# MarcKloter/bulletproofs_gadgets

Measured on AMD Instinct MI355X. Metric: R1CS constraints/sec (prove), 2^20-constraint MiMC-Merkle, 1/2/4/8 GPU, higher is better.
Workload: dtype u32

## Files before the change

### bulletproofs_gadgets_amd/csrc/engine.hip

```cpp
#include <hip/hip_runtime.h>
#include <algorithm>
#include <array>
#include <chrono>
#include <cerrno>
#include <cstdio>
#include <cstdlib>
#include <cstring>
#include <atomic>
#include <condition_variable>
#include <deque>
#include <functional>
#include <map>
#include <memory>
#include <mutex>
#include <thread>
#include <sched.h>
#include <fcntl.h>
#include <sys/stat.h>
#include <unistd.h>
#include "engine.hpp"
#include "hip_handles.hpp"
#include "host/fe51.hpp"
#include "host/chain.hpp"
#include "host/fiat_shamir.hpp"
#include "host/csc_work.hpp"
#include "host/verify_wave_plan.hpp"
#include "host/merkle_plan.hpp"
#include "hip/kernels.cuh"

namespace bpg {

#define BPG_LAUNCH_ID(I, id, kernel, grid, block, ...) do { (I).prof_begin(id); hipLaunchKernelGGL(kernel, grid, block, 0, (I).st, __VA_ARGS__); (I).prof_end(id); } while (0)
#define BPG_LAUNCH(I, kernel, grid, block, ...) BPG_LAUNCH_ID(I, KID_##kernel, kernel, grid, block, __VA_ARGS__)
#define BPG_LAUNCH_LDS(I, id, kernel, grid, block, lds, ...) do { (I).prof_begin(id); hipLaunchKernelGGL(kernel, grid, block, lds, (I).st, __VA_ARGS__); (I).prof_end(id); } while (0)

namespace {

static std::mutex g_table_bytes_mutex;
static std::map<int, uint64_t> g_table_bytes;
static uint64_t table_bytes_held(int device) { std::lock_guard<std::mutex> lk(g_table_bytes_mutex); return g_table_bytes[device]; }
static void table_bytes_add(int device, int64_t delta) { std::lock_guard<std::mutex> lk(g_table_bytes_mutex); g_table_bytes[device] = (uint64_t)((int64_t)g_table_bytes[device] + delta); }
static std::atomic<int> g_proving[64];
struct ProvingGuard {
    std::atomic<int> &c;
    explicit ProvingGuard(int device) : c(g_proving[(unsigned)device & 63u]) { c.fetch_add(1, std::memory_order_relaxed); }
    ~ProvingGuard() { c.fetch_sub(1, std::memory_order_relaxed); }
};
static bool device_shared(int device) { return g_proving[(unsigned)device & 63u].load(std::memory_order_relaxed) > 1; }
struct SharedTables {
    int device = 0; uint64_t cap = 0;
    DevBuf gens;
    std::mutex m;
    std::map<uint32_t, DevBuf> wide;
    std::map<uint32_t, DevBuf> odd;
    std::map<uint64_t, uint64_t> refused;
    ~SharedTables() {
        (void)hipSetDevice(device);
        uint64_t held = 0;
        for (auto &kv : odd) held += kv.second.cap;
        for (auto &kv : wide) held += kv.second.cap;
        table_bytes_add(device, -(int64_t)held);
    }
};
struct MimcConstants {
    int device = 0; DevBuf rc;
    ~MimcConstants() { (void)hipSetDevice(device); }
};
static std::mutex g_mimc_mutex;
void merkle_orphan(DeviceMerkle *t);
static std::map<int, std::weak_ptr<MimcConstants>> g_mimc;
static std::mutex g_tables_mutex;
// ... 127 lines not shown
    void prof_note(int id, double alg_bytes, double act_bytes, double fm) { if (!prof_on(id)) return; prof_alg_bytes[id] += alg_bytes; prof_act_bytes[id] += act_bytes; prof_fm[id] += fm; }
    void prof_collect() {
        if (prof_open.empty()) return;
        HIPCHK(hipStreamSynchronize(st));
        for (ProfRec &r : prof_open) { float ms = 0; HIPCHK(hipEventElapsedTime(&ms, r.a, r.b)); prof_ms[r.id] += ms; prof_count[r.id]++; if ((r.id == KID_k_witness_eval || r.id == KID_k_witness_eval_repeat || r.id == KID_k_witness_eval_join) && prof_wit_ms.size() < 1024) prof_wit_ms.push_back(ms); if ((r.id == KID_k_merkle_level || r.id == KID_k_merkle_top || r.id == KID_k_merkle_level_list || r.id == KID_k_merkle_level_range || r.id == KID_k_merkle_climb) && prof_merkle_ms.size() < 512) prof_merkle_ms.emplace_back(r.id, ms); prof_pool.push_back(std::move(r.a)); prof_pool.push_back(std::move(r.b)); }
        prof_open.clear();
    }
    void prof_reset() { prof_collect(); for (int i = 0; i < KID_COUNT; i++) { prof_ms[i] = 0; prof_count[i] = 0; prof_alg_bytes[i] = prof_act_bytes[i] = prof_fm[i] = 0; } prof_wit_ms.clear(); prof_merkle_ms.clear(); }
    std::shared_ptr<SharedTables> shared;
    const ge_niels *gens = nullptr;
    DevBuf bases, scratch_ext, comp, small_in, small_sc;
    std::shared_ptr<MimcConstants> mimc;
    DevBuf mk_in, mk_out;
    std::vector<DeviceMerkle *> trees;
    DevBuf chk_v, chk_bitmap, chk_report;
    DevBuf ck_first;
    uint32_t check_threshold = CHECK_ROW_THRESHOLD;
    void rowview_build(DeviceCircuit *c);
    void fill_input_slots(DeviceCircuit *c);
    DevBuf arena;
    uint8_t *arena_at(size_t off) const { return arena.as<uint8_t>() + off; }
    bool blocking_waits = false;
    void wait_stream() {
        if (blocking_waits && !shared_now) {
            const double until = now_ms() + 3.0;
            do {
                const hipError_t e = hipStreamQuery(st);
                if (e == hipSuccess) return;
                if (e != hipErrorNotReady) HIPCHK(e);
                for (int k = 0; k < 64; k++) __builtin_ia32_pause();
            } while (now_ms() < until);
        }
        HIPCHK(hipStreamSynchronize(st));
    }
    static size_t al256(size_t x) { return (x + 255) & ~(size_t)255; }
    DevBuf counts, starts, cursor, blocksum, buckets, partial, msm_result, open_keys, medium, wsums, wq_stage, wq_tickets, tile_hist, heavy, plain, starts1;
    uint32_t sweep_blocks_resident = 1024;
    uint32_t msm_cmax = 15;
    uint32_t msm_cmax_shared = 16;
    uint32_t rseg = 8;
    uint32_t lgch = 0;
    bool gens_share = true;
    uint32_t profile = 1;
    bool shared_now = false;
    uint32_t msm_cmin = 2;
    uint32_t wit_waves = 1024;
    uint32_t merge_equal = 1;
    uint32_t merged_last = 0, merged_skipped_last = 0;
    void merge_witness(DeviceCircuit *c, const ge_niels *Gtab, const ge_niels *Htab);
    void merge_build(DeviceCircuit::MergeSet &M, const scm *A, const ge_niels *PA, uint32_t nA, const scm *B, const ge_niels *PB, uint32_t nB);
    double merge_ms_last = 0;
    DevBuf sLR, yinvpow, lv, rv, red_partial, red_out, raw_rng, extras;
    DevBuf stale_flag;
    DevBuf ipa_s, ipa_tabA, ipa_tabB, naf, qsteps, vfy_in, vfy_pts, vfy_ok, vfy_sc, vfy_ch;
    DevBuf vfy_small;
    DevBuf vw_raw, vw_flags, vw_standing, vw_tail1;
    uint32_t cu_count = 256;
    DevBuf tt_bases, tt_table, tt_f, tt_c, tt_partial, grp_c, ped_table, s_parts;
    uint32_t tt_orig_M0 = 0; const void *tt_orig_gens = nullptr;
    ge_pniels *tt_table_p = nullptr;
    void tt_build(const ge_niels *G, const ge_niels *H, const ge_niels *B, uint32_t M0, bool original) {
        const uint32_t npts = 2 * M0 + 1;
        if (original && tt_orig_M0 == M0 && tt_orig_gens == gens) { tt_table_p = tt_table.as<ge_pniels>(); return; }
        const size_t bb = al256((size_t)npts * TT_WINDOWS * sizeof(ge_ext)), tb = (size_t)npts * TT_WINDOWS * TT_MULTS * sizeof(ge_pniels);
        ge_ext *basesp;
        if (original) {
            tt_orig_M0 = 0;
// ... 85 lines not shown
                BPG_LAUNCH((*this), k_normalize_niels, ngrid, dim3(256), base.as<ge_ext>(), tab0, cnt);
                BPG_LAUNCH((*this), k_odd_start_ext, grid, dim3(256), base.as<ge_ext>(), scratch_ext.as<ge_ext>(), dbl.as<ge_ext>(), cnt);
            }
            for (uint32_t m = 1; m < NM; m++) {
                if (m > 1) BPG_LAUNCH((*this), k_odd_step, grid, dim3(256), scratch_ext.as<ge_ext>(), dbl.as<ge_ext>(), cnt);
                BPG_LAUNCH((*this), k_normalize_niels, ngrid, dim3(256), scratch_ext.as<ge_ext>(), tab0 + (size_t)m * cnt, cnt);
            }
        }
        HIPCHK(hipGetLastError());
        HIPCHK(hipStreamSynchronize(st));
        } catch (...) {
            (void)hipStreamSynchronize(st); table_bytes_add(shared->device, -(int64_t)odd.cap);
            throw;
        }
        gens_odd = (shared->odd[key_built] = std::move(odd)).as<ge_niels>();
        return true;
    }
    uint32_t fold_split_max = 65536;
    uint32_t fold_adapt = 1;
    bool shared_variants() const { return fold_adapt == 2 || (fold_adapt == 1 && device_shared(shared->device)); }
    bool fold_quad = true;
    bool fold_quad_w = true;
    bool fold_reg_w = true;
    FoldKnobs fold_knobs() const {
        FoldKnobs k;
        k.fold_wnaf = fold_wnaf; k.fold_split_max = fold_split_max; k.fold_quad = fold_quad; k.fold_quad_w = fold_quad_w; k.fold_reg_w = fold_reg_w; k.shared = shared_now;
        return k;
    }
    bool window_quad = true;
    uint32_t window_quad_blocks = 288;
    uint32_t fold_group = 3;
    uint32_t tt_lg = 12;
    uint32_t tt_orig_lg = 14;
    uint32_t batch_wave_mb = 512;
    DevBuf bt_dev; PinBuf bt_pin;
    uint32_t commit_cpw = 4;
    Event commit_ev;
    PinBuf h_raw, h_small;
    using BlindStream = bpg::BlindStream;
    using ChainWorker = bpg::ChainWorker;
    std::shared_ptr<ChainWorker> chain;
    uint32_t pool_streams = 0;
    uint32_t chain_workers = 1;
    uint32_t chain_lanes = 1;
    std::deque<std::shared_ptr<BlindStream>> blinds;
    std::vector<std::shared_ptr<BlindStream>> slab_owner;
    std::vector<PinBuf> h_blind;
    struct SlabDev { Stream copy_st; DevBuf d; std::vector<Event> ev; };
    static hipEvent_t block_event(const BlindStream &bs, uint64_t k) { return (*static_cast<const std::vector<Event> *>(bs.ev))[k]; }
// ... 14 lines not shown
    }
    void blind_release(const std::shared_ptr<BlindStream> &b) {
        blind_stop(b);
        for (auto it = blinds.begin(); it != blinds.end(); ++it) if (it->get() == b.get()) { blinds.erase(it); break; }
    }
    void blind_cancel() {
        while (!blinds.empty()) { blind_retire(blinds.front()); blinds.pop_front(); }
    }
    void chain_shutdown() {
        blind_cancel();
        if (!chain) return;
        if (!chain->pool) chain->stop();
        chain.reset(); pool_streams = 0;
    }
    uint64_t gens_cap = 0;
    DevBuf gens_load_cached(const std::string &path, uint64_t cap);
    void adopt(const std::shared_ptr<SharedTables> &sp) { shared = sp; gens = sp->gens.as<ge_niels>(); gens_cap = sp->cap; gens_odd = nullptr; }
    void gens_store_cached(const std::string &path, uint64_t cap);

    struct MsmTicket { uint32_t slot, nmsm, W; };
    static constexpr uint32_t WS_SLOTS = 8, WS_SLOT_BYTES = (uint32_t)MSM_WS_SLOT_BYTES;
    PinBuf h_wsums; uint32_t ws_next = 0;
    MsmTicket msm(const MsmJob &J, uint32_t nmsm);
    MsmKnobs msm_knobs() const {
        MsmKnobs k;
        k.cmin = msm_cmin; k.cmax = msm_cmax; k.cmax_shared = msm_cmax_shared; k.rseg = rseg; k.lgch = lgch; k.sweep_blocks_resident = sweep_blocks_resident;
        k.window_quad = window_quad; k.window_quad_blocks = window_quad_blocks; k.shared = shared_now;
        return k;
    }
    MsmRun msm_last{};
    DevBuf test_skip;
    DevBuf test_fold_tab;
    std::vector<h51::pt> msm_points(const MsmTicket &t) const {
        std::vector<h51::pt> out(t.nmsm);
        const uint32_t *w = reinterpret_cast<const uint32_t *>(h_wsums.as<uint8_t>() + (size_t)t.slot * WS_SLOT_BYTES);
        for (uint32_t m = 0; m < t.nmsm; m++) out[m] = h51::pt_horner(w + (size_t)m * t.W * 32, t.W);
        return out;
    }
    PinBuf stage; Event stage_ev[2];
    void h2d(void *dst, const void *src, size_t bytes) {
        const size_t SLOT = 8u << 20;
        stage.ensure(2 * SLOT);
        for (int k = 0; k < 2; k++) if (!stage_ev[k]) stage_ev[k] = Event::untimed();
        const uint8_t *s8 = static_cast<const uint8_t *>(src); uint8_t *d8 = static_cast<uint8_t *>(dst);
        int slot = 0;
        for (size_t off = 0; off < bytes; off += SLOT, slot ^= 1) {
            const size_t len = std::min(SLOT, bytes - off);
            HIPCHK(hipEventSynchronize(stage_ev[slot]));
            std::memcpy(stage.as<uint8_t>() + (size_t)slot * SLOT, s8 + off, len);
            HIPCHK(hipMemcpyAsync(d8 + off, stage.as<uint8_t>() + (size_t)slot * SLOT, len, hipMemcpyHostToDevice, st));
// ... 85 lines not shown
    }
    K->chain_workers = cfg.chain_workers ? cfg.chain_workers : 1u; if (!cfg.chain_workers) env_set("BPG_CHAIN_WORKERS", 1, 64, K->chain_workers);
    K->chain_lanes = cfg.chain_lanes ? cfg.chain_lanes : 1u; if (!cfg.chain_lanes) env_set("BPG_CHAIN_LANES", 1, 8, K->chain_lanes);
    K->gens_cache_dir = cfg.gens_cache_dir;
    if (K->gens_cache_dir.empty()) { if (const char *e = std::getenv("BPG_GENS_CACHE_DIR")) K->gens_cache_dir = e; }
    if (env_present("BPG_MSM_CMAX")) K->msm_cmax = K->msm_cmax_shared = (uint32_t)env_int_strict("BPG_MSM_CMAX", 4, 16);
    env_set("BPG_MSM_CMIN", 2, 16, K->msm_cmin);
    env_set("BPG_MERGE", 0, 2, K->merge_equal);
    bool resident_set = false;
    if (env_present("BPG_SWEEP_RESIDENT")) { K->sweep_blocks_resident = (uint32_t)env_int_strict("BPG_SWEEP_RESIDENT", 64, 65536); resident_set = true; }
    if (env_present("BPG_RSEG")) {
        const long v = env_int_strict("BPG_RSEG", 1, 1024);
        if (v & (v - 1)) throw std::invalid_argument("BPG_RSEG: the segment length of the bucket reduction is a power of two in [1, 1024]");
        K->rseg = (uint32_t)v;
    }
    env_set("BPG_LGCH", 2, 10, K->lgch);
    env_set("BPG_FOLD_SPLIT", 0, 1 << 24, K->fold_split_max);
    if (env_present("BPG_FOLD_QUAD")) K->fold_quad = env_int_strict("BPG_FOLD_QUAD", 0, 1) != 0;
    if (env_present("BPG_FOLD_QUAD_W")) K->fold_quad_w = env_int_strict("BPG_FOLD_QUAD_W", 0, 1) != 0;
    if (env_present("BPG_FOLD_REG_W")) K->fold_reg_w = env_int_strict("BPG_FOLD_REG_W", 0, 1) != 0;
    if (env_present("BPG_WINDOW_QUAD")) K->window_quad = env_int_strict("BPG_WINDOW_QUAD", 0, 1) != 0;
    env_set("BPG_WINDOW_QUAD_BLOCKS", 1, 65536, K->window_quad_blocks);
    env_set("BPG_FOLD_ADAPT", 0, 2, K->fold_adapt);
    env_set("BPG_FOLD_GROUP", 1, 5, K->fold_group);
    if (env_present("BPG_TT_WIDE_GB")) K->tt_wide_budget = (uint64_t)(env_double_strict("BPG_TT_WIDE_GB", 0.0, 4096.0) * (double)(1ull << 30));
    if (env_present("BPG_FOLD_TABLE_GB")) K->fold_table_budget = (uint64_t)(env_double_strict("BPG_FOLD_TABLE_GB", 0.0, 4096.0) * (double)(1ull << 30));
    if (env_present("BPG_FOLD_PARTS")) { const long v = env_int_strict("BPG_FOLD_PARTS", 1, 8); if (v & (v - 1)) throw std::invalid_argument("BPG_FOLD_PARTS: 1, 2, 4 or 8"); K->fold_parts = (uint32_t)v; }
    if (env_present("BPG_FOLD_WNAF")) { const long v = env_int_strict("BPG_FOLD_WNAF", 0, 8); if (v == 1 || v == 2) throw std::invalid_argument("BPG_FOLD_WNAF: 0 (register kernels) or 3..8"); K->fold_wnaf = (uint32_t)v; }
    if (env_present("BPG_TT_LG")) K->tt_lg = K->tt_orig_lg = (uint32_t)env_int_strict("BPG_TT_LG", 0, 20);
    env_set("BPG_TT_ORIG_LG", 0, 20, K->tt_orig_lg);
    env_set("BPG_BATCH_WAVE_MB", 0, 1 << 20, K->batch_wave_mb);
    env_set("BPG_COMMIT_CPW", 1, 4, K->commit_cpw);
    env_set("BPG_CHECK_THRESHOLD", 0, 1 << 20, K->check_threshold);
    if (env_present("BPG_GENS_SHARE")) K->gens_share = env_int_strict("BPG_GENS_SHARE", 0, 1) != 0;

    int count = 0;
    hipError_t e = hipGetDeviceCount(&count);
    if (e != hipSuccess || count <= 0) throw DeviceError("no HIP device available: the bpg engine has no CPU path");
    if (device < 0 || device >= count) throw DeviceError("invalid device ordinal");
    HIPCHK(hipSetDevice(device));
    if (blocking == 1) { (void)hipSetDeviceFlags(hipDeviceScheduleBlockingSync); (void)hipGetLastError(); K->blocking_waits = true; }
    {
        int cus = 0;
        if (hipDeviceGetAttribute(&cus, hipDeviceAttributeMultiprocessorCount, device) == hipSuccess && cus > 0) {
            if (!resident_set) K->sweep_blocks_resident = (uint32_t)cus * 4u;
            K->wit_waves = (uint32_t)cus * 4u;
// ... 31 lines not shown
Engine::Impl::~Impl() {
    chain_shutdown();
    if (!st) return;
    (void)hipSetDevice(device);
    (void)hipStreamSynchronize(st);
    for (auto &sd : slab_dev) if (sd->copy_st) (void)hipStreamSynchronize(sd->copy_st);
    for (DeviceMerkle *t : trees) merkle_orphan(t);
}

void live_resources(uint64_t out[6]) { for (int k = 0; k < LIVE_COUNT; k++) out[k] = g_live[k].load(std::memory_order_relaxed); }
int Engine::device_count() { int n = 0; if (hipGetDeviceCount(&n) != hipSuccess) { (void)hipGetLastError(); return 0; } return n; }
void Engine::profile_set(int mode) { HIPCHK(hipSetDevice(device_)); impl_->prof_reset(); impl_->prof_mode = mode; }
std::string Engine::profile_report() {
    HIPCHK(hipSetDevice(device_));
    impl_->prof_collect();
    char sch[1024];
    std::snprintf(sch, sizeof sch, "{\"_schedule\": {\"profile\": %u, \"tt_lg\": %u, \"tt_orig_lg\": %u, \"fold_group\": %u, \"fold_wnaf\": %u, \"fold_parts\": %u, "
                  "\"eff_wnaf\": %u, \"eff_parts\": %u, \"fold_adapt\": %u, \"fold_split_max\": %u, \"fold_quad\": %u, \"msm_cmax\": %u, \"msm_cmax_shared\": %u, \"msm_cmin\": %u, "
                  "\"rseg\": %u, \"lgch\": %u, \"sweep_blocks_resident\": %u, \"shared_variants_last\": %u, \"merge_equal\": %u, \"merged_last\": %u, \"merged_skipped_last\": %u, \"merge_ms_last\": %.3f, \"table_budget\": %llu, \"table_bytes\": %llu, \"check_threshold\": %u}",
                  impl_->profile, impl_->tt_lg, impl_->tt_orig_lg, impl_->fold_group, impl_->fold_wnaf, impl_->fold_parts, impl_->eff_wnaf, impl_->eff_parts,
                  impl_->fold_adapt, impl_->fold_split_max, (unsigned)impl_->fold_quad, impl_->msm_cmax, impl_->msm_cmax_shared, impl_->msm_cmin, impl_->rseg, impl_->lgch,
                  impl_->sweep_blocks_resident, (unsigned)impl_->shared_now, (unsigned)impl_->merge_equal, impl_->merged_last, impl_->merged_skipped_last, impl_->merge_ms_last, (unsigned long long)impl_->table_budget, (unsigned long long)table_bytes_held(device_), impl_->check_threshold);
    std::string out = sch;
    if (!impl_->prof_wit_ms.empty()) {
        out += ", \"_witness_launch_ms\": [";
        for (size_t i = 0; i < impl_->prof_wit_ms.size(); i++) { char b[32]; std::snprintf(b, sizeof b, "%s%.4f", i ? "," : "", impl_->prof_wit_ms[i]); out += b; }
        out += "]";
    }
    if (!impl_->prof_merkle_ms.empty()) {
        out += ", \"_merkle_launch_ms\": [";
        for (size_t i = 0; i < impl_->prof_merkle_ms.size(); i++) {
            char b[64]; std::snprintf(b, sizeof b, "%s[\"%s\", %.4f]", i ? "," : "", kKernelNames[impl_->prof_merkle_ms[i].first], impl_->prof_merkle_ms[i].second); out += b;
        }
        out += "]";
    }
    bool first = false;
    for (int i = 0; i < KID_COUNT; i++) {
        if (!impl_->prof_count[i]) continue;
        char buf[512];
        std::snprintf(buf, sizeof buf, "%s\"%s\": {\"count\": %llu, \"total_ms\": %.6f, \"alg_bytes\": %.0f, \"device_bytes\": %.0f, \"field_mults\": %.0f}",
                      first ? "" : ", ", kKernelNames[i], (unsigned long long)impl_->prof_count[i], impl_->prof_ms[i], impl_->prof_alg_bytes[i],
                      impl_->prof_act_bytes[i], impl_->prof_fm[i]);
        out += buf; first = false;
    }
    return out + "}";
}
// ... 188 lines not shown
}

void Engine::pedersen_commit(size_t k, const uint8_t *v, const uint8_t *blind, uint8_t *out) {
    if (!k) return;
    HIPCHK(hipSetDevice(device_));
    Impl &I = *impl_;
    std::vector<uint8_t> hv(k * 32), hr(k * 32);
    for (size_t i = 0; i < k; i++) {
        Scalar a = Scalar::from_bits(v + 32 * i); a.to_bytes(&hv[32 * i]);
        Scalar b = Scalar::from_bytes_mod_order(blind + 32 * i); b.to_bytes(&hr[32 * i]);
    }
    I.small_sc.ensure(2 * k * 32); I.comp.ensure(k * 32);
    HIPCHK(hipMemcpyAsync(I.small_sc.p, hv.data(), k * 32, hipMemcpyHostToDevice, I.st));
    HIPCHK(hipMemcpyAsync(I.small_sc.as<uint8_t>() + k * 32, hr.data(), k * 32, hipMemcpyHostToDevice, I.st));
    BPG_LAUNCH(I, k_pedersen, dim3((uint32_t)k), dim3(64), I.small_sc.as<uint32_t>(), I.small_sc.as<uint32_t>() + k * 8,
                       I.ped_table.as<ge_pniels>(), I.comp.as<uint8_t>(), (uint32_t)k);
    HIPCHK(hipGetLastError());
    HIPCHK(hipMemcpyAsync(out, I.comp.p, k * 32, hipMemcpyDeviceToHost, I.st));
    HIPCHK(hipStreamSynchronize(I.st));
}

Engine::Impl::MsmTicket Engine::Impl::msm(const MsmJob &J, uint32_t nmsm) {
    const MsmSegs &S = J.S;
    const MsmRun R = plan_msm(MsmShape{S.nseg, S.len, S.msm, nmsm, J.skipped}, msm_knobs());
    const MsmPlan &P = R.P;
    const uint32_t total = R.total, W = P.W, nkeys = R.nkeys, nchunks = R.nchunks, CH = R.CH;
    msm_last = R;
    starts.ensure(R.bytes_starts);
    buckets.ensure(R.bytes_buckets);
    partial.ensure(R.bytes_partial);
    arena.ensure(R.b_front + R.b_entries);
    uint16_t *digits_p = reinterpret_cast<uint16_t *>(arena_at(0));
    uint32_t *entries1_p = reinterpret_cast<uint32_t *>(arena_at(R.b_digits)), *entries_p = reinterpret_cast<uint32_t *>(arena_at(R.b_front));
    ge_ext *slotA = reinterpret_cast<ge_ext *>(arena_at(0)), *slotB = slotA + nchunks;
    heavy.ensure(R.bytes_heavy); medium.ensure(R.bytes_medium);
    counts.ensure(R.bytes_counts); starts1.ensure(R.bytes_counts); cursor.ensure(R.bytes_counts);
    blocksum.ensure(R.bytes_blocksum);
    HIPCHK(hipMemsetAsync(counts.p, 0, (size_t)R.nflat * 4, st));
    BPG_LAUNCH_LDS((*this), KID_k_msm_digits, k_msm_digits, dim3(R.ntiles ? R.ntiles : 1), dim3(512), R.lds_digits, S, P, total, digits_p, counts.as<uint32_t>(), heavy.as<uint32_t>(), medium.as<uint32_t>());
    BPG_LAUNCH((*this), k_scan_blocksums, dim3(R.nblk1), dim3(256), counts.as<uint32_t>(), R.nflat, blocksum.as<uint32_t>());
    BPG_LAUNCH((*this), k_scan_apply, dim3(R.nblk1), dim3(256), counts.as<uint32_t>(), R.nflat, blocksum.as<uint32_t>(), starts1.as<uint32_t>(), cursor.as<uint32_t>());
    if (R.ntiles) BPG_LAUNCH((*this), k_msm_scatter1, dim3(R.ntiles, W), dim3(256), S, P, digits_p, total, starts1.as<uint32_t>(), entries1_p);
    BPG_LAUNCH((*this), k_msm_sort2, dim3(R.K), dim3(256), P, starts1.as<uint32_t>(), R.nflat, entries1_p, starts.as<uint32_t>(), entries_p);
    open_keys.ensure(R.bytes_open_keys);
    BPG_LAUNCH((*this), k_bucket_chunks, dim3(cdiv(nchunks, 256)), dim3(256), S, starts.as<uint32_t>(), entries_p,
               buckets.as<ge_ext>(), slotA, slotB, open_keys.as<uint32_t>(), nkeys, CH);
    prof_note(KID_k_bucket_chunks, 64.0 * (double)(total - std::min(total, J.alg_discount)), 100.0 * (double)R.Mub, 7.0 * (double)R.Mub);
    if (!R.per_bucket)
        BPG_LAUNCH((*this), k_bucket_combine, dim3(cdiv(nchunks, 256)), dim3(256), starts.as<uint32_t>(), buckets.as<ge_ext>(), slotA, slotB, open_keys.as<uint32_t>(), nkeys, CH, heavy.as<uint32_t>(), medium.as<uint32_t>());
    else
        BPG_LAUNCH_ID((*this), KID_k_bucket_combine, k_bucket_combine_per_bucket, dim3(cdiv(nkeys, 256)), dim3(256), starts.as<uint32_t>(), buckets.as<ge_ext>(), slotA, slotB, nkeys, CH, heavy.as<uint32_t>());
    BPG_LAUNCH((*this), k_bucket_combine_heavy, dim3(HEAVY_BLOCKS), dim3(256), starts.as<uint32_t>(), buckets.as<ge_ext>(), slotA, slotB, CH, heavy.as<uint32_t>(), medium.as<uint32_t>());
    BPG_LAUNCH((*this), k_bucket_reduce, dim3(cdiv(R.nred, 64)), dim3(64), buckets.as<ge_ext>(), starts.as<uint32_t>(), partial.as<ge_ext>(), P.nb, R.seg, R.nsegpw, R.nred);
    wsums.ensure(R.bytes_wsums);
    if (R.quad) {
        wq_stage.ensure(R.bytes_wq_stage);
        if (!wq_tickets.p) { wq_tickets.ensure(MSM_TICKETS * 4); HIPCHK(hipMemsetAsync(wq_tickets.p, 0, MSM_TICKETS * 4, st)); }
        BPG_LAUNCH((*this), k_window_sums_quad, dim3(R.window_blocks, nmsm * W), dim3(256), partial.as<ge_ext>(), wsums.as<ge_ext>(), wq_stage.as<ge_ext>(), wq_tickets.as<uint32_t>(), R.nsegpw, R.nred,
                   ceil_log2(R.seg), R.lgper);
    } else
        BPG_LAUNCH((*this), k_window_sums, dim3(nmsm * W), dim3(R.window_threads), partial.as<ge_ext>(), wsums.as<ge_ext>(), R.nsegpw, R.nred, ceil_log2(R.seg));
    HIPCHK(hipGetLastError());
    h_wsums.ensure((size_t)WS_SLOTS * WS_SLOT_BYTES);
    MsmTicket t{ws_next, nmsm, W};
    ws_next = (ws_next + 1) % WS_SLOTS;
    HIPCHK(hipMemcpyAsync(h_wsums.as<uint8_t>() + (size_t)t.slot * WS_SLOT_BYTES, wsums.p, R.bytes_wsums, hipMemcpyDeviceToHost, st));
    return t;
}

void Engine::msm_gens(uint64_t first, uint64_t count, const uint8_t *s, const uint8_t *t, uint8_t out[32]) {
    if (first + count > gens_cap_) throw std::invalid_argument("msm_gens: range beyond capacity");
    HIPCHK(hipSetDevice(device_));
    Impl &I = *impl_;
    I.shared_now = I.shared_variants();
    I.small_sc.ensure(2 * count * 32 + 64); I.sLR.ensure(2 * count * sizeof(scm) + 64);
    I.msm_result.ensure(4 * sizeof(ge_ext)); I.comp.ensure(128);
    if (count) {
        HIPCHK(hipMemcpyAsync(I.small_sc.p, s, count * 32, hipMemcpyHostToDevice, I.st));
        HIPCHK(hipMemcpyAsync(I.small_sc.as<uint8_t>() + count * 32, t, count * 32, hipMemcpyHostToDevice, I.st));
        BPG_LAUNCH(I, k_sc_from_bytes, dim3(cdiv(2 * count, 256)), dim3(256), I.small_sc.as<uint32_t>(), I.sLR.as<scm>(), (uint32_t)(2 * count));
// ... 1107 lines not shown
    BPG_LAUNCH((*this), k_merge_sum, dim3(cdiv(groups, 64)), dim3(64), T, count, moff, goff, gslot, members, groups, scratch_ext.as<ge_ext>(), M.sc.as<scm>());
    BPG_LAUNCH((*this), k_normalize_niels, dim3(cdiv(cdiv(groups, NORM_K), 256)), dim3(256), scratch_ext.as<ge_ext>(), M.pts.as<ge_niels>(), groups);
    HIPCHK(hipGetLastError());
    if (merge_equal != 2) HIPCHK(hipStreamSynchronize(st));
    M.groups = groups; M.skipped = skipped;
}
void Engine::Impl::merge_witness(DeviceCircuit *c, const ge_niels *Gtab, const ge_niels *Htab) {
    if (c->merge_tried) return;
    c->merge_tried = true;
    const uint32_t n = (uint32_t)c->n;
    if (!merge_equal || n < 2) return;
    const double t0 = now_ms();
    merge_build(c->mI, c->aL.as<scm>(), Gtab, n, c->aR.as<scm>(), Htab, n);
    merge_build(c->mO, c->aO.as<scm>(), Gtab, n, nullptr, nullptr, 0);
    merge_ms_last = now_ms() - t0;
}

Engine::Impl::FoldRun Engine::Impl::fold_launch(const FoldShape &shape, const FoldKernel *forced, uint64_t g_M, uint64_t n, const Scalar &u_ch,
                                               const std::vector<Scalar> &sG, const std::vector<Scalar> &sH, const ge_niels *Gst, const ge_niels *Hst, ge_niels *dst) {
    Impl &I = *this;
    const uint32_t Mr = shape.Mr, nterms = shape.nterms;
    const bool g_first = shape.first;
    I.scratch_ext.ensure((size_t)2 * Mr * sizeof(ge_ext));
    const FoldKnobs knobs = I.fold_knobs();
    const FoldKernel kernel = forced ? *forced : choose_fold(shape, knobs, fold_wants_tables(shape, knobs) && I.odd_ensure());
    static const int kid_of[] = {KID_k_fold_points_wnaf, KID_k_fold_points_quadw, KID_k_fold_points_quad, KID_k_fold_points_split, KID_k_fold_points_regw,
                                 KID_k_fold_points_reg, KID_k_fold_points};
    const int fold_kid = kid_of[(int)kernel];
    const dim3 grid(cdiv(2 * Mr, 256)), grid64(cdiv(2 * Mr, 64)), block(256);
    ge_ext *fo = I.scratch_ext.as<ge_ext>();
    FoldRecode rc; FoldWnaf fw; FoldQuadW fq; FoldGroup fg;
    const bool wnaf = kernel == FoldKernel::Wnaf, steps = kernel == FoldKernel::QuadW || kernel == FoldKernel::RegW;
    PinBuf &hbuf = steps ? I.h_qsteps : I.h_naf;
    DevBuf &dbuf = steps ? I.qsteps : I.naf;
    const size_t bytes = wnaf ? fold_wnaf_bytes(nterms, I.eff_parts) : steps ? (size_t)2 * QW_MAXSTEPS * 4 : fold_naf_words(nterms) * 4;
    hbuf.ensure(bytes); dbuf.ensure(bytes);
    FoldRun run{kernel, -1, {0, 0}, {0, 0}};
    if (wnaf) {
        rc = fold_recode_wnaf(sG, sH, u_ch, Mr, n, g_first, I.eff_wnaf, I.eff_parts, I.fold_part_bits(), hbuf.as<int8_t>());
        fw.Mr = Mr; fw.nterms = nterms; fw.first_group = g_first; fw.n = (uint32_t)n; fw.cap = (uint32_t)gens_cap; fw.top = rc.top;
        fw.parts = I.eff_parts; fw.NM = 1u << (I.eff_wnaf - 2);
        run.top = fw.top;
    } else if (steps) {
        rc = fold_recode_steps(sG, sH, Mr, hbuf.as<uint32_t>(), fq);
        I.arena.ensure((size_t)3 * nterms * 2 * Mr * sizeof(ge_pniels));
        for (int c = 0; c < 2; c++) { run.nsteps[c] = fq.nsteps[c]; run.tail[c] = fq.tail[c]; }
    } else {
        rc = fold_recode_naf(sG, sH, u_ch, Mr, n, g_first, hbuf.as<uint32_t>());
// ... 74 lines not shown
    wait_stream();
    for (int k = 0; k < 3; k++) h51::pt_compress(pts + 32 * k, h51::pt_from_device(hp + 32 * k));
}

void Engine::Impl::inner_product(Transcript &T, std::vector<uint8_t> &proof, uint64_t n, uint64_t N, const Scalar &yinv, const Scalar &u_ch,
                                 const Scalar &w, const ge_niels *Gtab, const ge_niels *Htab, const ge_niels *Bn, ProveTimings *tm, double &t0) {
    Impl &I = *this;
    const uint32_t lgN = ceil_log2(N);
    auto lap = [&](double *slot) { if (tm) { I.wait_stream(); double t1 = now_ms(); *slot += t1 - t0; t0 = t1; } };
    T.innerproduct_domain_sep(N);
    std::vector<Scalar> yinv_pow2(lgN + 1);
    yinv_pow2[0] = yinv; for (uint32_t k = 1; k <= lgN; k++) yinv_pow2[k] = yinv_pow2[k - 1] * yinv_pow2[k - 1];
    scm *a = I.lv.as<scm>(), *b = I.rv.as<scm>();
    if (lgN) {
        const uint64_t half = N / 2;
        I.ipa_s.ensure(4 * half * sizeof(scm));
        I.ipa_tabA.ensure(2 * half * sizeof(ge_niels)); I.ipa_tabB.ensure((half > 1 ? half : 2) * sizeof(ge_niels));
        I.naf.ensure(4096);
    }
    Scalar Gamma = Scalar::one(), Eta = Scalar::one();
    const ge_niels *Gst = Gtab, *Hst = Htab;
    const scm w_m = to_scm(w), uch_m = to_scm(u_ch);
    uint64_t mcur = N;
    const uint32_t quad_sums = I.shared_now ? 0u : 1u;
    bool tt_on = false; Impl::TailState tt;
    const uint32_t GRP_STRIDE = 64;
    uint32_t g_j = 0, g_r = 1, g_cur = 0, g_index = 0; uint64_t g_M = N; bool g_first = true; std::vector<Scalar> g_us;
    for (uint32_t round = 0; round < lgN; round++) {
        const uint64_t h = mcur / 2;
        const bool first = round == 0;
        if (!tt_on && ((I.tt_lg > 0 && mcur <= (1ull << I.tt_lg)) || (first && I.tt_orig_lg > 0 && mcur <= (1ull << I.tt_orig_lg)))) {
            tt_on = true;
            const bool original = Gst == Gtab && Hst == Htab;
            I.tail_freeze(tt, (uint32_t)mcur, first, n, uch_m, Gamma, Eta, Gst, Hst, Bn, original, original && Gtab == I.gens);
        }
        if (tt_on) {
            uint8_t lr[64];
            I.tail_round(tt, a, b, mcur, w_m, quad_sums, lr);
            lap(tm ? &tm->ipa_msm : nullptr);
            proof.insert(proof.end(), lr, lr + 64);
            I.tail_challenge(tt, fs_ipa_round(T, lr, lr + 32));
            mcur = h;
            if (round + 1 == lgN) I.tail_last_fold(tt, a, b, h);
            continue;
        }
        if (g_j == 0) {
            g_M = mcur; g_first = first;
            uint32_t left = ceil_log2(mcur);
            if (I.tt_lg > 0 && left > I.tt_lg) left -= I.tt_lg;
            g_r = std::min<uint32_t>(I.fold_group, left);
            g_us.clear();
            I.grp_c.ensure(4 * GRP_STRIDE * sizeof(scm));
            g_cur = 0;
            hipLaunchKernelGGL(k_set2, dim3(1), dim3(64), 0, st, I.grp_c.as<scm>(), (uint32_t)GRP_STRIDE, to_scm(Gamma), to_scm(Eta));
        }
        scm *c0 = I.grp_c.as<scm>() + (size_t)g_cur * 2 * GRP_STRIDE;
        const uint64_t cnt = g_M / 2;
        scm *sLG = I.ipa_s.as<scm>(), *sLH = sLG + cnt, *sRG = sLH + cnt, *sRH = sRG + cnt;
        const uint32_t blocks = std::min<uint32_t>(cdiv(cnt, 256), 1024);
        const uint32_t lgh = ceil_log2(h);
        I.red_partial.ensure((size_t)blocks * 2 * sizeof(scm) + 4096);
// ... 125 lines not shown
    impl_->chain_shutdown();
    impl_->chain_workers = n;
}
void Engine::set_chain_lanes(uint32_t n) {
    if (n < 1 || n > 8) throw std::invalid_argument("chain lanes: 1..8");
    impl_->chain_shutdown();
    impl_->chain_lanes = n;
}
void Engine::blinding_cancel() { impl_->blind_cancel(); }
void Engine::test_fail_next_upload() { impl_->test_fail_upload = 1; }
void Engine::test_drop_next_upload() { impl_->test_fail_upload = 2; }
uint64_t Engine::table_bytes() const { return table_bytes_held(device_); }

int Engine::chain_cpu() const { return impl_->last_chain_cpu; }
bool Engine::last_shared_variants() const { return impl_->shared_now; }

std::vector<uint8_t> Engine::prove(DeviceCircuit *c, Transcript &T, const std::vector<Scalar> &v_blinding,
                                   const uint8_t rng_seed[32], uint32_t flags, ProveTimings *tm) {
    HIPCHK(hipSetDevice(device_));
    Impl &I = *impl_;
    hipStream_t st = I.st;
    ProvingGuard in_flight(device_);
    I.shared_now = I.shared_variants();
    if (tm) tm->shared_variants = I.shared_now ? 1u : 0u;
    const uint64_t n = c->n, m = c->m, q = c->q;
    if (v_blinding.size() != m) throw std::invalid_argument("prove: need one blinding factor per committed variable");
    if (!c->has_witness) throw R1CSException(R1CSError::MissingAssignment, "prove: the uploaded circuit carries no assignments (verifier-side instance)");
    const uint64_t N = padded_size(n);
    const uint32_t lgN = ceil_log2(N);
    require_gens_capacity(gens_cap_, n);
    const double t_begin = now_ms();
    double t0 = t_begin;
    auto lap = [&](double *slot) { if (tm) { I.wait_stream(); double t1 = now_ms(); *slot += t1 - t0; t0 = t1; } };

    const ge_niels *Gtab = I.gens, *Htab = I.gens + gens_cap_;
    const ge_niels *Bn = I.bases.as<ge_niels>(), *Bbn = Bn + 1;

    T.append_u64("m", m);
    const bool expanded = (flags & 4u) != 0;
    std::shared_ptr<Impl::BlindStream> bs;
    if (!I.blinds.empty()) {
        uint8_t now[203]; T.export_state(now);
        for (const std::shared_ptr<Impl::BlindStream> &cand : I.blinds) {
            const Impl::BlindStream &b = *cand;
            bool ok = !expanded && 2 * n <= b.max_draws && std::memcmp(now, b.state, 203) == 0 && std::memcmp(rng_seed, b.seed, 32) == 0 && b.vb.size() == v_blinding.size();
            for (size_t i = 0; ok && i < b.vb.size(); i++) ok = std::memcmp(b.vb[i].as_bytes(), v_blinding[i].as_bytes(), 32) == 0;
            if (ok) { bs = cand; break; }
// ... 97 lines not shown
                const uint64_t k = i / Impl::BlindStream::UP;
                while (bs->uploaded_blocks.load(std::memory_order_acquire) <= k) std::this_thread::sleep_for(std::chrono::microseconds(40));
                upload_failed();
                HIPCHK(hipStreamWaitEvent(st, Impl::block_event(*bs, k), 0));
            } else {
                rng.fill_draws64(raw + 64 * i, cnt);
                HIPCHK(hipMemcpyAsync(I.raw_rng.as<uint8_t>() + 64 * i, raw + 64 * i, cnt * 64, hipMemcpyHostToDevice, st));
            }
            if (!merged && i + cnt < 2 * n && next_piece < 3 && pieces[next_piece].b <= i + cnt) { convert_to(i + cnt); launch_pieces(i + cnt); }
        }
        convert_to(2 * n);
        }
    }
    if (bs) {
        const uint64_t K = (2 * n) / Impl::BlindStream::SNAP, rem = 2 * n - K * Impl::BlindStream::SNAP;
        while (bs->produced.load(std::memory_order_acquire) < K * Impl::BlindStream::SNAP) std::this_thread::sleep_for(std::chrono::microseconds(20));
        rng = bs->snaps[K];
        if (rem) { std::vector<uint8_t> skip(rem * 64); rng.fill_draws64(skip.data(), rem); }
        I.blind_release(bs);
        { const int c = bs->cpu.load(std::memory_order_relaxed); if (c >= 0) I.last_chain_cpu = c; }
        bs.reset();
    }
    if (tm) tm->rng_host += now_ms() - t_rng0;
    lap(tm ? &tm->msm_aiao : nullptr);
    uint8_t pts[96];
    if (tabled) {
        I.commit3(c->aL.as<scm>(), c->aR.as<scm>(), c->aO.as<scm>(), sL, sR, n, (uint32_t)N, I.shared_now ? 0u : 1u, pts);
    } else if (merged) {
        MsmJob J = job_new();
        push_AI(J); push_AO(J);
        seg_push(J, sL, Gtab, (uint32_t)n, 2);
        seg_push(J, sR, Htab, (uint32_t)n, 2);
        seg_push(J, I.extras.as<scm>() + 2, Bbn, 1, 2);
        const Impl::MsmTicket tk = I.msm(J, 3);
        I.wait_stream();
        const std::vector<h51::pt> P3 = I.msm_points(tk);
        for (int k = 0; k < 3; k++) h51::pt_compress(pts + 32 * k, P3[k]);
    } else {
        launch_pieces(2 * n);
        I.wait_stream();
        const std::vector<h51::pt> AB = I.msm_points(tk_aiao);
        h51::pt Sp = I.msm_points(tk_s[0])[0];
        for (uint32_t k = 1; k < nparts; k++) Sp = h51::pt_add(Sp, I.msm_points(tk_s[k])[0]);
        h51::pt_compress(pts, AB[0]); h51::pt_compress(pts + 32, AB[1]); h51::pt_compress(pts + 64, Sp);
    }
    lap(tm ? &tm->msm_s : nullptr);

    std::vector<uint8_t> proof;
    proof_open(proof, lgN, flags, pts);
    Scalar y, z;
// ... 24 lines not shown
    if (*h_stale) {
        HIPCHK(hipMemsetAsync(I.stale_flag.p, 0, 4, st));
        throw DeviceError("a blinding draw was read before it was uploaded (stale device slab): proof withheld");
    }
    Scalar t[7], tb[7];
    for (int k = 0; k < 6; k++) t[k + 1] = from_scm(h_t[k]);
    Scalar u_ch, x;
    uint8_t vv[5 * 32], rr[5 * 32], tcom[5 * 32];
    poly_commit_inputs(rng, t, tb, vv, rr);
    pedersen_commit(5, vv, rr, tcom);
    fs_poly_commitments(T, tcom, u_ch, x);
    proof.insert(proof.end(), tcom, tcom + 160);
    const PolyAtX px = poly_at_x(t, tb, [&](uint64_t j) { return from_scm(h_wV[j]); }, v_blinding, ib, ob, sb, x);
    const Scalar w = fs_poly_scalars(T, px.tx, px.txb, px.eb);
    proof_poly_scalars(proof, px);

    I.lv.ensure(N * sizeof(scm)); I.rv.ensure(N * sizeof(scm));
    BPG_LAUNCH(I, k_poly_eval, dim3(cdiv(N, 256)), dim3(256), c->aL.as<scm>(), c->aR.as<scm>(), c->aO.as<scm>(), sL, sR, wL, wR, wO,
                       ypow_p, I.yinvpow.as<scm>(), to_scm(x), I.lv.as<scm>(), I.rv.as<scm>(), (uint32_t)n, (uint32_t)N);
    HIPCHK(hipGetLastError());
    lap(tm ? &tm->poly : nullptr);

    I.inner_product(T, proof, n, N, yinv, u_ch, w, Gtab, Htab, Bn, tm, t0);
    if (tm) { tm->ipa = tm->ipa_msm + tm->ipa_fold; tm->total += now_ms() - t_begin; }
    return proof;
}

namespace {
uint32_t batch_host_threads() {
    cpu_set_t set; CPU_ZERO(&set);
    long n = sched_getaffinity(0, sizeof set, &set) == 0 ? CPU_COUNT(&set) : 1;
    if (FILE *f = std::fopen("/sys/fs/cgroup/cpu.max", "r")) {
        char quota[32] = {0}; long period = 0;
        if (std::fscanf(f, "%31s %ld", quota, &period) == 2 && std::strcmp(quota, "max") != 0 && period > 0) n = std::min(n, std::max(1L, (std::atol(quota) + period - 1) / period));
        std::fclose(f);
    }
    return (uint32_t)std::max(1L, std::min(n, 16L));
}
class StageThreads {
public:
    explicit StageThreads(uint32_t n) { for (uint32_t t = 1; t < n; t++) th_.emplace_back([this] { loop(); }); }
    ~StageThreads() { { std::lock_guard<std::mutex> lk(mu_); quit_ = true; } cv_.notify_all(); for (std::thread &t : th_) t.join(); }
    void run(size_t count, const std::function<void(size_t, size_t)> &fn) {
        const size_t parts = std::min<size_t>(count, 4 * (th_.size() + 1));
        if (parts <= 1 || th_.empty()) { if (count) fn(0, count); return; }
        { std::lock_guard<std::mutex> lk(mu_); fn_ = &fn; count_ = count; parts_ = parts; next_.store(0); busy_.store((int)th_.size()); gen_++; }
        cv_.notify_all();
// ... 1221 lines not shown
```

Measured before the change: 84.96 million.

## Choose lone or shared kernel variants per proving stage using device fill gauge

```diff
diff --git a/bulletproofs_gadgets_amd/csrc/engine.hip b/bulletproofs_gadgets_amd/csrc/engine.hip
--- a/bulletproofs_gadgets_amd/csrc/engine.hip
+++ b/bulletproofs_gadgets_amd/csrc/engine.hip
@@ -26,6 +26,7 @@
 #include "host/csc_work.hpp"
 #include "host/verify_wave_plan.hpp"
 #include "host/merkle_plan.hpp"
+#include "host/fill_policy.hpp"
 #include "hip/kernels.cuh"
 
 namespace bpg {
@@ -47,6 +48,18 @@
     ~ProvingGuard() { c.fetch_sub(1, std::memory_order_relaxed); }
 };
 static bool device_shared(int device) { return g_proving[(unsigned)device & 63u].load(std::memory_order_relaxed) > 1; }
+static std::atomic<int> g_past_chain[64];
+struct PastChainGuard {
+    std::atomic<int> *c = nullptr;
+    bool *flag = nullptr;
+    PastChainGuard() = default;
+    PastChainGuard(const PastChainGuard &) = delete;
+    PastChainGuard &operator=(const PastChainGuard &) = delete;
+    void enter(int device, bool *in_flag) { if (c) return; c = &g_past_chain[(unsigned)device & 63u]; c->fetch_add(1, std::memory_order_relaxed); flag = in_flag; *flag = true; }
+    ~PastChainGuard() { if (c) { c->fetch_sub(1, std::memory_order_relaxed); *flag = false; } }
+};
+static uint32_t fill_gauge(int device) { const int v = g_past_chain[(unsigned)device & 63u].load(std::memory_order_relaxed); return v > 0 ? (uint32_t)v : 0u; }
+static uint32_t proofs_in_flight(int device) { const int v = g_proving[(unsigned)device & 63u].load(std::memory_order_relaxed); return v > 0 ? (uint32_t)v : 0u; }
 struct SharedTables {
     int device = 0; uint64_t cap = 0;
     DevBuf gens;
@@ -220,14 +233,14 @@
     uint8_t *arena_at(size_t off) const { return arena.as<uint8_t>() + off; }
     bool blocking_waits = false;
     void wait_stream() {
-        if (blocking_waits && !shared_now) {
+        if (blocking_waits && !stage_shared(FillStage::Wait)) {
             const double until = now_ms() + 3.0;
             do {
                 const hipError_t e = hipStreamQuery(st);
                 if (e == hipSuccess) return;
                 if (e != hipErrorNotReady) HIPCHK(e);
                 for (int k = 0; k < 64; k++) __builtin_ia32_pause();
-            } while (now_ms() < until);
+            } while (now_ms() < until && !stage_peek(FillStage::Wait));
         }
         HIPCHK(hipStreamSynchronize(st));
     }
@@ -241,6 +254,29 @@
     bool gens_share = true;
     uint32_t profile = 1;
     bool shared_now = false;
+    FillKnobs fill;
+    std::string fill_pattern;
+    bool per_stage = false, past_chain = false, first_decided = false;
+    uint32_t fill_decisions = 0;
+    uint32_t stage_taken[FILL_STAGES][2] = {};
+    bool stage_peek(FillStage s) const {
+        if (!per_stage) return shared_now;
+        return variant_for(s, past_chain ? fill_gauge(device) : proofs_in_flight(device), fill) == FillVariant::Shared;
+    }
+    bool stage_shared(FillStage s) {
+        if (!per_stage) return shared_now;
+        const bool forced = fill.fold_adapt == 1 && s != FillStage::Wait && !fill_pattern.empty();
+        const bool sh = forced ? fill_pattern_at(fill_pattern, fill_decisions++) == FillVariant::Shared : stage_peek(s);
+        stage_taken[(uint32_t)s][sh ? 1 : 0]++;
+        if (s != FillStage::Wait && !first_decided) { first_decided = true; shared_now = sh; }
+        return sh;
+    }
+    FillStage msm_stage() const { return past_chain ? FillStage::Msm : FillStage::ChainMsm; }
+    struct StageScope {
+        Impl &I;
+        explicit StageScope(Impl &i) : I(i) { I.per_stage = true; I.first_decided = false; I.fill_decisions = 0; std::memset(I.stage_taken, 0, sizeof I.stage_taken); }
+        ~StageScope() { I.per_stage = false; }
+    };
     uint32_t msm_cmin = 2;
     uint32_t wit_waves = 1024;
     uint32_t merge_equal = 1;
@@ -372,9 +408,9 @@
     bool fold_quad = true;
     bool fold_quad_w = true;
     bool fold_reg_w = true;
-    FoldKnobs fold_knobs() const {
+    FoldKnobs fold_knobs(bool shared_variant) const {
         FoldKnobs k;
-        k.fold_wnaf = fold_wnaf; k.fold_split_max = fold_split_max; k.fold_quad = fold_quad; k.fold_quad_w = fold_quad_w; k.fold_reg_w = fold_reg_w; k.shared = shared_now;
+        k.fold_wnaf = fold_wnaf; k.fold_split_max = fold_split_max; k.fold_quad = fold_quad; k.fold_quad_w = fold_quad_w; k.fold_reg_w = fold_reg_w; k.shared = shared_variant;
         return k;
     }
     bool window_quad = true;
@@ -435,10 +471,10 @@
     static constexpr uint32_t WS_SLOTS = 8, WS_SLOT_BYTES = (uint32_t)MSM_WS_SLOT_BYTES;
     PinBuf h_wsums; uint32_t ws_next = 0;
     MsmTicket msm(const MsmJob &J, uint32_t nmsm);
-    MsmKnobs msm_knobs() const {
+    MsmKnobs msm_knobs(bool shared_variant) const {
         MsmKnobs k;
         k.cmin = msm_cmin; k.cmax = msm_cmax; k.cmax_shared = msm_cmax_shared; k.rseg = rseg; k.lgch = lgch; k.sweep_blocks_resident = sweep_blocks_resident;
-        k.window_quad = window_quad; k.window_quad_blocks = window_quad_blocks; k.shared = shared_now;
+        k.window_quad = window_quad; k.window_quad_blocks = window_quad_blocks; k.shared = shared_variant;
         return k;
     }
     MsmRun msm_last{};
@@ -570,6 +606,16 @@
     if (env_present("BPG_WINDOW_QUAD")) K->window_quad = env_int_strict("BPG_WINDOW_QUAD", 0, 1) != 0;
     env_set("BPG_WINDOW_QUAD_BLOCKS", 1, 65536, K->window_quad_blocks);
     env_set("BPG_FOLD_ADAPT", 0, 2, K->fold_adapt);
+    K->fill.fold_adapt = K->fold_adapt;
+    {
+        static const char *const names[FILL_STAGES] = {"BPG_FILL_CHAIN_MSM", "BPG_FILL_MSM", "BPG_FILL_FOLD", "BPG_FILL_TAIL", "BPG_FILL_WAIT"};
+        for (uint32_t s = 0; s < FILL_STAGES; s++) env_set(names[s], 0, FILL_THRESHOLD_MAX, K->fill.threshold[s]);
+        fill_knobs_check(K->fill);
+        if (env_present("BPG_FILL_PATTERN")) {
+            K->fill_pattern = std::getenv("BPG_FILL_PATTERN");
+            if (!fill_pattern_valid(K->fill_pattern)) throw std::invalid_argument("BPG_FILL_PATTERN=" + K->fill_pattern + ": expected 1..4096 letters l (lone) and s (shared)");
+        }
+    }
     env_set("BPG_FOLD_GROUP", 1, 5, K->fold_group);
     if (env_present("BPG_TT_WIDE_GB")) K->tt_wide_budget = (uint64_t)(env_double_strict("BPG_TT_WIDE_GB", 0.0, 4096.0) * (double)(1ull << 30));
     if (env_present("BPG_FOLD_TABLE_GB")) K->fold_table_budget = (uint64_t)(env_double_strict("BPG_FOLD_TABLE_GB", 0.0, 4096.0) * (double)(1ull << 30));
@@ -647,6 +693,17 @@
                   impl_->fold_adapt, impl_->fold_split_max, (unsigned)impl_->fold_quad, impl_->msm_cmax, impl_->msm_cmax_shared, impl_->msm_cmin, impl_->rseg, impl_->lgch,
                   impl_->sweep_blocks_resident, (unsigned)impl_->shared_now, (unsigned)impl_->merge_equal, impl_->merged_last, impl_->merged_skipped_last, impl_->merge_ms_last, (unsigned long long)impl_->table_budget, (unsigned long long)table_bytes_held(device_), impl_->check_threshold);
     std::string out = sch;
+    {
+        std::string fill_s;
+        for (uint32_t s = 0; s < FILL_STAGES; s++) {
+            char b[192]; const char *nm = fill_stage_name((FillStage)s);
+            std::snprintf(b, sizeof b, ", \"fill_%s\": %u, \"stages_%s_lone_last\": %u, \"stages_%s_shared_last\": %u", nm, impl_->fill.threshold[s], nm, impl_->stage_taken[s][0], nm, impl_->stage_taken[s][1]);
+            fill_s += b;
+        }
+        char b[64]; std::snprintf(b, sizeof b, ", \"fill_gauge_now\": %u", fill_gauge(device_));
+        fill_s += b;
+        out.insert(out.size() - 1, fill_s);
+    }
     if (!impl_->prof_wit_ms.empty()) {
         out += ", \"_witness_launch_ms\": [";
         for (size_t i = 0; i < impl_->prof_wit_ms.size(); i++) { char b[32]; std::snprintf(b, sizeof b, "%s%.4f", i ? "," : "", impl_->prof_wit_ms[i]); out += b; }
@@ -881,27 +938,34 @@
 
 Engine::Impl::MsmTicket Engine::Impl::msm(const MsmJob &J, uint32_t nmsm) {
     const MsmSegs &S = J.S;
-    const MsmRun R = plan_msm(MsmShape{S.nseg, S.len, S.msm, nmsm, J.skipped}, msm_knobs());
+    const MsmShape shape{S.nseg, S.len, S.msm, nmsm, J.skipped};
+    const MsmKnobs knobs = msm_knobs(stage_shared(msm_stage()));
+    const MsmRun R = plan_msm(shape, knobs);
     const MsmPlan &P = R.P;
     const uint32_t total = R.total, W = P.W, nkeys = R.nkeys, nchunks = R.nchunks, CH = R.CH;
     msm_last = R;
-    starts.ensure(R.bytes_starts);
-    buckets.ensure(R.bytes_buckets);
-    partial.ensure(R.bytes_partial);
-    arena.ensure(R.b_front + R.b_entries);
+    const MsmWorkspace ws = msm_workspace_either(shape, knobs, fill.fold_adapt == 1, R);
+    starts.ensure(ws.starts);
+    buckets.ensure(ws.buckets);
+    partial.ensure(ws.partial);
+    arena.ensure(ws.arena);
     uint16_t *digits_p = reinterpret_cast<uint16_t *>(arena_at(0));
     uint32_t *entries1_p = reinterpret_cast<uint32_t *>(arena_at(R.b_digits)), *entries_p = reinterpret_cast<uint32_t *>(arena_at(R.b_front));
     ge_ext *slotA = reinterpret_cast<ge_ext *>(arena_at(0)), *slotB = slotA + nchunks;
-    heavy.ensure(R.bytes_heavy); medium.ensure(R.bytes_medium);
-    counts.ensure(R.bytes_counts); starts1.ensure(R.bytes_counts); cursor.ensure(R.bytes_counts);
-    blocksum.ensure(R.bytes_blocksum);
+    heavy.ensure(ws.heavy); medium.ensure(ws.medium);
+    counts.ensure(ws.counts); starts1.ensure(ws.counts); cursor.ensure(ws.counts);
+    blocksum.ensure(ws.blocksum);
+    open_keys.ensure(ws.open_keys); wsums.ensure(ws.wsums);
+    if (ws.wq_stage) {
+        wq_stage.ensure(ws.wq_stage);
+        if (!wq_tickets.p) { wq_tickets.ensure(MSM_TICKETS * 4); HIPCHK(hipMemsetAsync(wq_tickets.p, 0, MSM_TICKETS * 4, st)); }
+    }
     HIPCHK(hipMemsetAsync(counts.p, 0, (size_t)R.nflat * 4, st));
     BPG_LAUNCH_LDS((*this), KID_k_msm_digits, k_msm_digits, dim3(R.ntiles ? R.ntiles : 1), dim3(512), R.lds_digits, S, P, total, digits_p, counts.as<uint32_t>(), heavy.as<uint32_t>(), medium.as<uint32_t>());
     BPG_LAUNCH((*this), k_scan_blocksums, dim3(R.nblk1), dim3(256), counts.as<uint32_t>(), R.nflat, blocksum.as<uint32_t>());
     BPG_LAUNCH((*this), k_scan_apply, dim3(R.nblk1), dim3(256), counts.as<uint32_t>(), R.nflat, blocksum.as<uint32_t>(), starts1.as<uint32_t>(), cursor.as<uint32_t>());
     if (R.ntiles) BPG_LAUNCH((*this), k_msm_scatter1, dim3(R.ntiles, W), dim3(256), S, P, digits_p, total, starts1.as<uint32_t>(), entries1_p);
     BPG_LAUNCH((*this), k_msm_sort2, dim3(R.K), dim3(256), P, starts1.as<uint32_t>(), R.nflat, entries1_p, starts.as<uint32_t>(), entries_p);
-    open_keys.ensure(R.bytes_open_keys);
     BPG_LAUNCH((*this), k_bucket_chunks, dim3(cdiv(nchunks, 256)), dim3(256), S, starts.as<uint32_t>(), entries_p,
                buckets.as<ge_ext>(), slotA, slotB, open_keys.as<uint32_t>(), nkeys, CH);
     prof_note(KID_k_bucket_chunks, 64.0 * (double)(total - std::min(total, J.alg_discount)), 100.0 * (double)R.Mub, 7.0 * (double)R.Mub);
@@ -911,10 +975,7 @@
         BPG_LAUNCH_ID((*this), KID_k_bucket_combine, k_bucket_combine_per_bucket, dim3(cdiv(nkeys, 256)), dim3(256), starts.as<uint32_t>(), buckets.as<ge_ext>(), slotA, slotB, nkeys, CH, heavy.as<uint32_t>());
     BPG_LAUNCH((*this), k_bucket_combine_heavy, dim3(HEAVY_BLOCKS), dim3(256), starts.as<uint32_t>(), buckets.as<ge_ext>(), slotA, slotB, CH, heavy.as<uint32_t>(), medium.as<uint32_t>());
     BPG_LAUNCH((*this), k_bucket_reduce, dim3(cdiv(R.nred, 64)), dim3(64), buckets.as<ge_ext>(), starts.as<uint32_t>(), partial.as<ge_ext>(), P.nb, R.seg, R.nsegpw, R.nred);
-    wsums.ensure(R.bytes_wsums);
     if (R.quad) {
-        wq_stage.ensure(R.bytes_wq_stage);
-        if (!wq_tickets.p) { wq_tickets.ensure(MSM_TICKETS * 4); HIPCHK(hipMemsetAsync(wq_tickets.p, 0, MSM_TICKETS * 4, st)); }
         BPG_LAUNCH((*this), k_window_sums_quad, dim3(R.window_blocks, nmsm * W), dim3(256), partial.as<ge_ext>(), wsums.as<ge_ext>(), wq_stage.as<ge_ext>(), wq_tickets.as<uint32_t>(), R.nsegpw, R.nred,
                    ceil_log2(R.seg), R.lgper);
     } else
@@ -2068,8 +2129,16 @@
     const uint32_t Mr = shape.Mr, nterms = shape.nterms;
     const bool g_first = shape.first;
     I.scratch_ext.ensure((size_t)2 * Mr * sizeof(ge_ext));
-    const FoldKnobs knobs = I.fold_knobs();
-    const FoldKernel kernel = forced ? *forced : choose_fold(shape, knobs, fold_wants_tables(shape, knobs) && I.odd_ensure());
+    const FoldKnobs knobs = I.fold_knobs(I.stage_shared(FillStage::Fold));
+    const bool tables = fold_wants_tables(shape, knobs) && I.odd_ensure();
+    const FoldKernel kernel = forced ? *forced : choose_fold(shape, knobs, tables);
+    if (!forced && I.fill.fold_adapt == 1) {
+        const FoldKernel other = choose_fold(shape, I.fold_knobs(!knobs.shared), tables);
+        if (other == FoldKernel::QuadW || other == FoldKernel::RegW) {
+            I.h_qsteps.ensure((size_t)2 * QW_MAXSTEPS * 4); I.qsteps.ensure((size_t)2 * QW_MAXSTEPS * 4);
+            I.arena.ensure((size_t)3 * nterms * 2 * Mr * sizeof(ge_pniels));
+        } else if (other != FoldKernel::Wnaf) { I.h_naf.ensure(fold_naf_words(nterms) * 4); I.naf.ensure(fold_naf_words(nterms) * 4); }
+    }
     static const int kid_of[] = {KID_k_fold_points_wnaf, KID_k_fold_points_quadw, KID_k_fold_points_quad, KID_k_fold_points_split, KID_k_fold_points_regw,
                                  KID_k_fold_points_reg, KID_k_fold_points};
     const int fold_kid = kid_of[(int)kernel];
@@ -2190,7 +2259,6 @@
     const ge_niels *Gst = Gtab, *Hst = Htab;
     const scm w_m = to_scm(w), uch_m = to_scm(u_ch);
     uint64_t mcur = N;
-    const uint32_t quad_sums = I.shared_now ? 0u : 1u;
     bool tt_on = false; Impl::TailState tt;
     const uint32_t GRP_STRIDE = 64;
     uint32_t g_j = 0, g_r = 1, g_cur = 0, g_index = 0; uint64_t g_M = N; bool g_first = true; std::vector<Scalar> g_us;
@@ -2204,7 +2272,7 @@
         }
         if (tt_on) {
             uint8_t lr[64];
-            I.tail_round(tt, a, b, mcur, w_m, quad_sums, lr);
+            I.tail_round(tt, a, b, mcur, w_m, I.stage_shared(FillStage::Tail) ? 0u : 1u, lr);
             lap(tm ? &tm->ipa_msm : nullptr);
             proof.insert(proof.end(), lr, lr + 64);
             I.tail_challenge(tt, fs_ipa_round(T, lr, lr + 32));
@@ -2376,7 +2444,8 @@
     hipStream_t st = I.st;
     ProvingGuard in_flight(device_);
     I.shared_now = I.shared_variants();
-    if (tm) tm->shared_variants = I.shared_now ? 1u : 0u;
+    Impl::StageScope stages(I);
+    PastChainGuard past_chain;
     const uint64_t n = c->n, m = c->m, q = c->q;
     if (v_blinding.size() != m) throw std::invalid_argument("prove: need one blinding factor per committed variable");
     if (!c->has_witness) throw R1CSException(R1CSError::MissingAssignment, "prove: the uploaded circuit carries no assignments (verifier-side instance)");
@@ -2520,10 +2589,11 @@
         bs.reset();
     }
     if (tm) tm->rng_host += now_ms() - t_rng0;
+    past_chain.enter(device_, &I.past_chain);
     lap(tm ? &tm->msm_aiao : nullptr);
     uint8_t pts[96];
     if (tabled) {
-        I.commit3(c->aL.as<scm>(), c->aR.as<scm>(), c->aO.as<scm>(), sL, sR, n, (uint32_t)N, I.shared_now ? 0u : 1u, pts);
+        I.commit3(c->aL.as<scm>(), c->aR.as<scm>(), c->aO.as<scm>(), sL, sR, n, (uint32_t)N, I.stage_shared(FillStage::Tail) ? 0u : 1u, pts);
     } else if (merged) {
         MsmJob J = job_new();
         push_AI(J); push_AO(J);
@@ -2594,7 +2664,7 @@
     lap(tm ? &tm->poly : nullptr);
 
     I.inner_product(T, proof, n, N, yinv, u_ch, w, Gtab, Htab, Bn, tm, t0);
-    if (tm) { tm->ipa = tm->ipa_msm + tm->ipa_fold; tm->total += now_ms() - t_begin; }
+    if (tm) { tm->ipa = tm->ipa_msm + tm->ipa_fold; tm->total += now_ms() - t_begin; tm->shared_variants = I.shared_now ? 1u : 0u; }
     return proof;
 }
 
diff --git a/bulletproofs_gadgets_amd/csrc/host/fill_policy.hpp b/bulletproofs_gadgets_amd/csrc/host/fill_policy.hpp
--- /dev/null
+++ b/bulletproofs_gadgets_amd/csrc/host/fill_policy.hpp
@@ -0,0 +1,73 @@
+#pragma once
+#include <algorithm>
+#include <cstdint>
+#include <stdexcept>
+#include <string>
+#include "msm_plan.hpp"
+
+namespace bpg {
+
+enum class FillStage : uint32_t {
+    ChainMsm = 0,
+    Msm,
+    Fold,
+    Tail,
+    Wait,
+    Count
+};
+constexpr uint32_t FILL_STAGES = (uint32_t)FillStage::Count;
+constexpr uint32_t FILL_THRESHOLD_MAX = 64;
+constexpr uint32_t FILL_COUNT_MAX = 0x7fffffffu;
+inline const char *fill_stage_name(FillStage s) {
+    static const char *const names[FILL_STAGES] = {"chain_msm", "msm", "fold", "tail", "wait"};
+    return names[(uint32_t)s];
+}
+
+enum class FillVariant : uint32_t { Lone = 0, Shared = 1 };
+
+struct FillKnobs {
+    uint32_t fold_adapt = 1;
+    uint32_t threshold[FILL_STAGES] = {2, 5, 5, 5, 5};
+};
+inline void fill_knobs_check(const FillKnobs &k) {
+    if (k.fold_adapt > 2) throw std::invalid_argument("fold_adapt: 0 (never), 1 (by the fill gauge) or 2 (always)");
+    for (uint32_t s = 0; s < FILL_STAGES; s++)
+        if (k.threshold[s] > FILL_THRESHOLD_MAX) throw std::invalid_argument(std::string("fill threshold of stage ") + fill_stage_name((FillStage)s) + ": 0.." + std::to_string(FILL_THRESHOLD_MAX));
+}
+inline FillVariant variant_for(FillStage stage, uint32_t proofs_loading, const FillKnobs &k) {
+    if (k.fold_adapt == 0) return FillVariant::Lone;
+    if (k.fold_adapt == 2) return FillVariant::Shared;
+    const uint32_t t = k.threshold[(uint32_t)stage];
+    return (t <= 1 || proofs_loading >= t) ? FillVariant::Shared : FillVariant::Lone;
+}
+
+inline bool fill_pattern_valid(const std::string &p) {
+    if (p.empty() || p.size() > 4096) return false;
+    for (char c : p) if (c != 'l' && c != 's') return false;
+    return true;
+}
+inline FillVariant fill_pattern_at(const std::string &p, uint32_t decision) { return p[decision % p.size()] == 's' ? FillVariant::Shared : FillVariant::Lone; }
+
+struct MsmWorkspace {
+    size_t arena, starts, buckets, partial, heavy, medium, counts, blocksum, open_keys, wsums, wq_stage;
+};
+inline MsmWorkspace msm_workspace(const MsmRun &R) {
+    return MsmWorkspace{R.b_front + R.b_entries, R.bytes_starts, R.bytes_buckets, R.bytes_partial, R.bytes_heavy, R.bytes_medium, R.bytes_counts, R.bytes_blocksum,
+                        R.bytes_open_keys, R.bytes_wsums, R.bytes_wq_stage};
+}
+inline MsmWorkspace msm_workspace_max(const MsmWorkspace &a, const MsmWorkspace &b) {
+    return MsmWorkspace{std::max(a.arena, b.arena), std::max(a.starts, b.starts), std::max(a.buckets, b.buckets), std::max(a.partial, b.partial), std::max(a.heavy, b.heavy),
+                        std::max(a.medium, b.medium), std::max(a.counts, b.counts), std::max(a.blocksum, b.blocksum), std::max(a.open_keys, b.open_keys),
+                        std::max(a.wsums, b.wsums), std::max(a.wq_stage, b.wq_stage)};
+}
+inline bool msm_workspace_covers(const MsmWorkspace &w, const MsmWorkspace &need) {
+    return w.arena >= need.arena && w.starts >= need.starts && w.buckets >= need.buckets && w.partial >= need.partial && w.heavy >= need.heavy && w.medium >= need.medium &&
+           w.counts >= need.counts && w.blocksum >= need.blocksum && w.open_keys >= need.open_keys && w.wsums >= need.wsums && w.wq_stage >= need.wq_stage;
+}
+inline MsmWorkspace msm_workspace_either(const MsmShape &S, const MsmKnobs &knobs, bool adaptive, const MsmRun &R) {
+    MsmWorkspace w = msm_workspace(R);
+    if (adaptive) { MsmKnobs other = knobs; other.shared = !knobs.shared; w = msm_workspace_max(w, msm_workspace(plan_msm(S, other))); }
+    return w;
+}
+
+}
```

New measurement: 85.48 million (median of 3 runs). No clear change (+0.6%).
